# jesusdpa1/ssqueeze_rs

Measured on AMD Instinct MI355X. Metric: TF-bins/sec (ssq_stft, n_fft=1024), higher is better.
Workload: dtype f32

## Files before the change

ssqueeze_rs_amd/csrc/stft_fused.hip:

```cpp
#include "stft_fused_kernel.h"

namespace ssq {

struct Hi1024 {
  static constexpr int N = 1024, L = 64, NF = 513, W = 16, F = 16, PITCH = F + 1, THREADS = W * 64;
  static constexpr int PLANE = NF * PITCH;
  static constexpr int TILE_BYTES = (((2 * PLANE + F) * 4 + 15) / 16) * 16;
  static constexpr int EXH_ELEMS = 64 * 9;
  static constexpr int EXH_BYTES = W * EXH_ELEMS * 8;
  static constexpr int TAB_BYTES = N * 8;
  static constexpr int LDS_BYTES = TILE_BYTES + EXH_BYTES + 2 * TAB_BYTES;
  static constexpr int FRAC = 30, EMIN = -90;
  static_assert(LDS_BYTES <= 160 * 1024, "LDS budget");
};

__device__ __forceinline__ void rows_transpose4(float& r0, float& r1, float& r2, float& r3) {
  auto a = __builtin_amdgcn_permlane32_swap(__float_as_uint(r0), __float_as_uint(r2), false, false);
  auto b = __builtin_amdgcn_permlane32_swap(__float_as_uint(r1), __float_as_uint(r3), false, false);
  auto c = __builtin_amdgcn_permlane16_swap(a[0], b[0], false, false);
  auto d = __builtin_amdgcn_permlane16_swap(a[1], b[1], false, false);
  r0 = __uint_as_float(c[0]);
  r1 = __uint_as_float(c[1]);
  r2 = __uint_as_float(d[0]);
  r3 = __uint_as_float(d[1]);
}

template <bool EDGE, bool LEB, bool WKDBG = false>
__global__ __launch_bounds__(1024, 1) void stft_tx1024_kernel(StftDev<float> p) {
  using H = Hi1024;
  constexpr int THREADS = H::THREADS;
  using T = float;
  constexpr int N = H::N, L = H::L, NF = H::NF, F = H::F, PITCH = H::PITCH;
  __shared__ __attribute__((aligned(16))) unsigned char smem[H::LDS_BYTES];
  int* tile_re = reinterpret_cast<int*>(smem);
  float* col_scale = reinterpret_cast<float*>(tile_re + 2 * H::PLANE);
  cpx<T>* exch_all = reinterpret_cast<cpx<T>*>(smem + H::TILE_BYTES);
  cpx<T>* win_lds = reinterpret_cast<cpx<T>*>(smem + H::TILE_BYTES + H::EXH_BYTES);
  cpx<T>* tw1 = win_lds + N;
  cpx<T>* tw2 = tw1 + 256;

  const int tid = threadIdx.x;
  const int t = tid & 63;
  const int fl = __builtin_amdgcn_readfirstlane(tid >> 6);
  cpx<T>* exch = exch_all + fl * H::EXH_ELEMS;

  for (int i = tid; i < N; i += THREADS) win_lds[i] = p.win2[i];
  if (tid < 256) tw1[tid] = p.tw[((tid & 15) * (tid >> 4) * 4) & (N - 1)];
  for (int i = tid; i < 768; i += THREADS) tw2[i] = p.tw[((i & 255) * ((i >> 8) + 1)) & (N - 1)];
  constexpr long long CELL0 = WKDBG ? 0LL : 0x80000000LL;
  for (int i = tid; i < H::PLANE; i += THREADS) reinterpret_cast<long long*>(tile_re)[i] = CELL0;
  __syncthreads();
  const unsigned bid = blockIdx.x;
  if ((long long)bid >= p.total_tiles) return;

  const long long n_sig = p.total_tiles / p.tiles_per_signal;
  long long sig = (long long)(bid / (unsigned)p.tiles_per_signal);
  int jt = (int)(bid % (unsigned)p.tiles_per_signal);
  auto tile_frame0 = [&](int j) { return ((j < p.ta_n) ? p.ta0 + j : p.tb0 + (j - p.ta_n)) * F; };
  auto load_frame = [&](long long sg, int frame0, T (&xv)[16]) {
    const int frame = frame0 + fl;
    const T* xs = sig_base(p, sg);
    const long long pos0 = (long long)frame * p.hop - p.pad_left + t;
    if constexpr (!EDGE) {
#pragma unroll
      for (int q = 0; q < 16; ++q) xv[q] = xs[pos0 + L * q];
    } else {
      const bool valid = frame < p.n_frames;
      const long long first = pos0 - t;
      if (__all(valid && first >= 0 && first + N <= p.n_signal)) {
#pragma unroll
        for (int q = 0; q < 16; ++q) xv[q] = xs[pos0 + L * q];
      } else {
#pragma unroll
        for (int q = 0; q < 16; ++q) xv[q] = load_padded_flat(xs, pos0 + L * q, p.n_signal, p.padtype, valid);
      }
    }
  };
  T xn[16];
  load_frame(sig, tile_frame0(jt), xn);
  const cpx<T> twr_unused[3][16] = {};

  auto read_out = [&](long long rsig, int rframe0) {
    if constexpr (!EDGE && !WKDBG) {
      if ((p.n_frames & 1) == 0) {
        constexpr int RS2 = THREADS / (F / 2);
        const int fp = tid % (F / 2);
        const int k0 = tid / (F / 2);
        float4* __restrict__ og4 = reinterpret_cast<float4*>(p.out + rsig * (long long)NF * p.n_frames + rframe0 + 2 * fp +
                                                             (long long)k0 * p.n_frames);
        const long long gstep4 = (long long)RS2 * p.n_frames / 2;
        const T sc0 = col_scale[2 * fp], sc1 = col_scale[2 * fp + 1];
        long long* tc = reinterpret_cast<long long*>(tile_re) + k0 * PITCH + 2 * fp;
        auto sweep2 = [&](int j) {
          const long long c0 = tc[j * RS2 * PITCH], c1 = tc[j * RS2 * PITCH + 1];
          tc[j * RS2 * PITCH] = CELL0;
          tc[j * RS2 * PITCH + 1] = CELL0;
          const int r0 = (int)c0 ^ (int)0x80000000, r1 = (int)c1 ^ (int)0x80000000;
          const int i0 = (int)(c0 >> 32), i1 = (int)(c1 >> 32);
          const float4 val = make_float4((T)r0 * sc0, (T)i0 * sc0, (T)r1 * sc1, (T)i1 * sc1);
          typedef float vf4 __attribute__((ext_vector_type(4)));
          const vf4 nv = {val.x, val.y, val.z, val.w};
          __builtin_nontemporal_store(nv, reinterpret_cast<vf4*>(&og4[j * gstep4]));
        };
        constexpr int NFULL2 = NF / RS2;
#pragma unroll
        for (int j = 0; j < NFULL2; ++j) sweep2(j);
        if (k0 + NFULL2 * RS2 < NF) sweep2(NFULL2);
        return;
      }
    }
    constexpr int RSTEP = THREADS / F;
    const int f = tid % F;
    const int k0 = tid / F;
    cpx<T>* __restrict__ og = p.out + rsig * (long long)NF * p.n_frames + rframe0 + f + (long long)k0 * p.n_frames;
    const long long gstep = (long long)RSTEP * p.n_frames;
    const bool fvalid = EDGE ? (rframe0 + f < p.n_frames) : true;
    const T sc = col_scale[f];
    constexpr int NFULL = NF / RSTEP;
    long long* tc = reinterpret_cast<long long*>(tile_re) + k0 * PITCH + f;
    auto sweep = [&](int j) {
      const long long c = tc[j * RSTEP * PITCH];
      tc[j * RSTEP * PITCH] = CELL0;
      if constexpr (WKDBG) {
        if (fvalid) og[j * gstep] = cpx<T>{__int_as_float((int)c), __int_as_float((int)(c >> 32))};
        return;
      }
      const int ire = (int)c ^ (int)0x80000000;
      const int iim = (int)(c >> 32);
      if (fvalid) og[j * gstep] = cpx<T>{(T)ire * sc, (T)iim * sc};
    };
#pragma unroll
    for (int j = 0; j < NFULL; ++j) sweep(j);
    if (k0 + NFULL * RSTEP < NF) sweep(NFULL);
  };

  const int grid_n = (int)gridDim.x;
#pragma unroll 1
  while (true) {
    const int frame0 = tile_frame0(jt);
    const bool valid = EDGE ? (frame0 + fl < p.n_frames) : true;
    long long nsig = sig;
    int njt = jt + grid_n;
    while (njt >= p.tiles_per_signal) {
      njt -= p.tiles_per_signal;
      ++nsig;
    }
    const bool has_next = nsig < n_sig;
    cpx<T> v[16];
#pragma unroll
    for (int q = 0; q < 16; ++q) {
      const cpx<T> wq = win_lds[t + L * q];
      v[q] = {xn[q] * wq.x, xn[q] * wq.y};
    }

    fft_compute<T, 10, 0, false, false>(v, twr_unused, tw1, t);
    {
      cpx<T> nv[16];
      const int rbase = 9 * (t >> 4) + (t & 7);
#pragma unroll
      for (int ph = 0; ph < 2; ++ph) {
#pragma unroll
        for (int u = 0; u < 8; ++u) exch[9 * t + u] = v[8 * ph + u];
        frame_sync<false>();
        if (((t >> 3) & 1) == ph) {
#pragma unroll
          for (int q = 0; q < 16; ++q) nv[q] = exch[rbase + 36 * q];
        }
        frame_sync<false>();
      }
#pragma unroll
      for (int q = 0; q < 16; ++q) v[q] = nv[q];
    }
    if (has_next) load_frame(nsig, tile_frame0(njt), xn);
    fft_compute<T, 10, 1, false, false, true>(v, twr_unused, tw1, t);
    {
#pragma unroll
      for (int uh = 0; uh < 4; ++uh) {
        rows_transpose4(v[4 * uh + 0].x, v[4 * uh + 1].x, v[4 * uh + 2].x, v[4 * uh + 3].x);
        rows_transpose4(v[4 * uh + 0].y, v[4 * uh + 1].y, v[4 * uh + 2].y, v[4 * uh + 3].y);
      }
#define SSQ_SWAP(i, j)       \
  {                          \
    const cpx<T> t_ = v[i];  \
    v[i] = v[j];             \
    v[j] = t_;               \
  }
      SSQ_SWAP(1, 4) SSQ_SWAP(2, 8) SSQ_SWAP(3, 12) SSQ_SWAP(6, 9) SSQ_SWAP(7, 13) SSQ_SWAP(11, 14)
#undef SSQ_SWAP
    }
    fft_compute<T, 10, 2, false, false, true>(v, twr_unused, tw2 - 256, t);

    cpx<T> zp[9];
    {
      const int src = (L - t) & (L - 1);
      zp[8] = v[8];
      if (t == 0) {
#pragma unroll
        for (int j = 8; j < 15; ++j) v[j] = v[j + 1];
        v[15] = v[0];
      }
#pragma unroll
      for (int q = 0; q < 8; ++q) {
        zp[q].x = __shfl(v[15 - q].x, src);
        zp[q].y = __shfl(v[15 - q].y, src);
      }
      v[8] = zp[8];
    }

    {
      cpx<T> cv[9];
      int dstb[9];
      T wdbg[9];
      int kdbg[9];
      T l1 = 0.0f;
      constexpr int CELL = 8;
      const float lane_on = valid ? 1.0f : 0.0f;
      const float sfs0 = (float)t * p.sfs_step, sfs_q = (float)L * p.sfs_step;
      const int neg_last = -(p.n_freqs - 1);
#pragma unroll
      for (int q = 0; q < 9; ++q) {
        const cpx<T> zk = v[q], zn = zp[q];
        const cpx<T> S = {zk.x + zn.x, zk.y - zn.y};
        const cpx<T> dS = {zk.y + zn.y, zn.x - zk.x};
        const float den = S.x * S.x + S.y * S.y;
        const float num = dS.y * S.x - dS.x * S.y;
        const float pd = num * __builtin_amdgcn_rcpf(den * p.two_pi_eff);
        const float d = (sfs0 + (float)q * sfs_q) - pd;
        const float w = fabsf(d);
        float m = fma_clamp01(den, p.keep_big, p.keep_bias) * fma_clamp01(d, 0.0f, 1.0f);
        if (EDGE) m *= lane_on;
        if (q == 8) m *= (t == 0) ? 1.0f : 0.0f;
        const cpx<T> c = LEB ? cpx<T>{p.leb_unit * m, 0.0f} : cpx<T>{S.x * m, S.y * m};
        cv[q] = c;
        int kneg = cvt_floor_i32(__builtin_fmaf(-w, p.inv_dw, 0.5f));
        kneg = kneg < neg_last ? neg_last : kneg;
        dstb[q] = __mul24(kneg, -(PITCH * CELL)) + fl * CELL;
        l1 += fabsf(c.x) + fabsf(c.y);
        if constexpr (WKDBG) {
          wdbg[q] = w;
          kdbg[q] = (m != 0.0f) ? -kneg : -1;
        }
      }
      const T tot = frame_allreduce<T, L, false>(l1, t, nullptr, t) * p.dw;
      T scale, inv_scale;
      column_scale<T, H::FRAC, H::EMIN>(tot, p.dw, scale, inv_scale);
      if (t == 0 && valid) col_scale[fl] = inv_scale;
      char* ptile = reinterpret_cast<char*>(tile_re);
      if constexpr (WKDBG) {
#pragma unroll
        for (int q = 0; q < 9; ++q) {
          if ((q < 8 || t == 0) && valid) {
            const unsigned lo = (unsigned)__float_as_int(wdbg[q]), hi = (unsigned)__float_as_int((float)kdbg[q]);
            reinterpret_cast<unsigned long long*>(ptile)[(t + L * q) * PITCH + fl] = ((unsigned long long)hi << 32) | lo;
          }
        }
      } else {
#pragma unroll
        for (int q = 0; q < 9; ++q) {
          const int ia = cvt_round_i32(cv[q].x * scale);
          const int ib = LEB ? 0 : cvt_round_i32(cv[q].y * scale);
          if (q < 8 || t == 0) {
            if (LEB) {
              atomicAdd(reinterpret_cast<unsigned*>(ptile + dstb[q]), (unsigned)ia);
            } else {
              const unsigned hi = (unsigned)(ib + (ia >> 31));
              atomicAdd(reinterpret_cast<unsigned long long*>(ptile + dstb[q]),
                        ((unsigned long long)hi << 32) | (unsigned)ia);
            }
          }
        }
      }
    }
    __syncthreads();
    read_out(sig, frame0);
    __syncthreads();
    if (!has_next) break;
    sig = nsig;
    jt = njt;
  }
}

template <typename T>
bool fused_supported(int n_fft) {
  return n_fft >= 64 && n_fft <= 4096 && (n_fft & (n_fft - 1)) == 0;
}

template <typename T, int LOGN>
static hipError_t launch_one(const StftDev<T>& p0, int cu_count, long long batch, hipStream_t stream) {
  using C = FusedCfg<T, LOGN>;
  int per_cu = (160 * 1024) / C::LDS_BYTES;
  if (per_cu < 1) per_cu = 1;
  if (per_cu * C::W > 32) per_cu = 32 / C::W;
  bool tx1024 = false;
  if constexpr (sizeof(T) == 4 && LOGN == 10) tx1024 = (p0.out_kind == 0 || p0.out_kind == 3) && p0.n_eff == C::N;
  const int TF = tx1024 ? Hi1024::F : C::F;
  const long long span = (long long)TF * p0.hop;
  const int tps_all = (p0.n_frames + TF - 1) / TF;
  long long lo = (p0.pad_left + span - 1) / span;
  long long hi_num = p0.n_signal - C::N - (long long)(TF - 1) * p0.hop + p0.pad_left;
  long long hi = hi_num >= 0 ? hi_num / span + 1 : 0;
  const long long full = p0.n_frames / TF;
  if (hi > full) hi = full;
  if (lo > tps_all) lo = tps_all;
  if (hi < lo) hi = lo;
  const long long blocks_one_wave = (long long)cu_count * (tx1024 ? 1 : per_cu);
  bool single_launch = (long long)tps_all * batch <= 4 * blocks_one_wave;
  if (const char* e = std::getenv("SSQ_SINGLE_LAUNCH")) single_launch = std::atoi(e) != 0;
  for (int edge = single_launch ? 1 : 0; edge < 2; ++edge) {
    StftDev<T> p = p0;
    if (single_launch) {
      p.ta0 = 0;
      p.ta_n = tps_all;
      p.tb0 = 0;
      p.tiles_per_signal = tps_all;
    } else if (!edge) {
      p.ta0 = (int)lo;
      p.ta_n = (int)(hi - lo);
      p.tb0 = 0;
      p.tiles_per_signal = p.ta_n;
    } else {
      p.ta0 = 0;
      p.ta_n = (int)lo;
      p.tb0 = (int)hi;
      p.tiles_per_signal = (int)lo + (tps_all - (int)hi);
    }
    p.total_tiles = (long long)p.tiles_per_signal * batch;
    if (p.total_tiles <= 0) continue;
    long long blocks = (long long)cu_count * per_cu;
    if (blocks > p.total_tiles) blocks = p.total_tiles;
    const dim3 g((unsigned)blocks), b(C::W * 64);
    if constexpr (sizeof(T) == 4 && LOGN == 10) {
      if (tx1024) {
        long long nb = cu_count;
        if (nb > p.total_tiles) nb = p.total_tiles;
        const dim3 gh((unsigned)nb), bh(Hi1024::THREADS);
        if (p.out_kind == 3) {
          if (edge) hipLaunchKernelGGL((stft_tx1024_kernel<true, false, true>), gh, bh, 0, stream, p);
          else hipLaunchKernelGGL((stft_tx1024_kernel<false, false, true>), gh, bh, 0, stream, p);
        } else if (p.squeezing == 1) {
          if (edge) hipLaunchKernelGGL((stft_tx1024_kernel<true, true>), gh, bh, 0, stream, p);
          else hipLaunchKernelGGL((stft_tx1024_kernel<false, true>), gh, bh, 0, stream, p);
        } else {
          if (edge) hipLaunchKernelGGL((stft_tx1024_kernel<true, false>), gh, bh, 0, stream, p);
          else hipLaunchKernelGGL((stft_tx1024_kernel<false, false>), gh, bh, 0, stream, p);
        }
        const hipError_t eh = hipGetLastError();
        if (eh != hipSuccess) return eh;
        continue;
      }
    }
    if (p.out_kind == 0 && p.squeezing == 1) {
      if (edge) hipLaunchKernelGGL((stft_fused_kernel<T, LOGN, true, true, true>), g, b, 0, stream, p);
      else hipLaunchKernelGGL((stft_fused_kernel<T, LOGN, true, false, true>), g, b, 0, stream, p);
    } else if (p.out_kind == 0) {
      if (edge) hipLaunchKernelGGL((stft_fused_kernel<T, LOGN, true, true, false>), g, b, 0, stream, p);
      else hipLaunchKernelGGL((stft_fused_kernel<T, LOGN, true, false, false>), g, b, 0, stream, p);
    } else if (p.out_kind == 3) {
      if (edge) hipLaunchKernelGGL((stft_fused_kernel<T, LOGN, true, true, false, true>), g, b, 0, stream, p);
      else hipLaunchKernelGGL((stft_fused_kernel<T, LOGN, true, false, false, true>), g, b, 0, stream, p);
    } else {
      if (edge) hipLaunchKernelGGL((stft_fused_kernel<T, LOGN, false, true, false>), g, b, 0, stream, p);
      else hipLaunchKernelGGL((stft_fused_kernel<T, LOGN, false, false, false>), g, b, 0, stream, p);
    }
    const hipError_t e = hipGetLastError();
    if (e != hipSuccess) return e;
  }
  return hipSuccess;
}

template <typename T>
int fused_tile_frames(int n_fft) {
  switch (n_fft) {
    case 64: return FusedCfg<T, 6>::F;
    case 128: return FusedCfg<T, 7>::F;
    case 256: return FusedCfg<T, 8>::F;
    case 512: return FusedCfg<T, 9>::F;
    case 1024: return FusedCfg<T, 10>::F;
    case 2048: return FusedCfg<T, 11>::F;
    case 4096: return FusedCfg<T, 12>::F;
  }
  return 0;
}

template <typename T>
hipError_t launch_stft_fused(const StftDev<T>& p, int n_fft, int cu_count, long long batch, hipStream_t stream) {
  if (p.n_eff != n_fft) return launch_stft_anylen<T>(p, n_fft, cu_count, batch, stream);
  switch (n_fft) {
    case 64: return launch_one<T, 6>(p, cu_count, batch, stream);
    case 128: return launch_one<T, 7>(p, cu_count, batch, stream);
    case 256: return launch_one<T, 8>(p, cu_count, batch, stream);
    case 512: return launch_one<T, 9>(p, cu_count, batch, stream);
    case 1024: return launch_one<T, 10>(p, cu_count, batch, stream);
    case 2048: return launch_one<T, 11>(p, cu_count, batch, stream);
    case 4096: return launch_one<T, 12>(p, cu_count, batch, stream);
  }
  return hipErrorInvalidValue;
}

template bool fused_supported<float>(int);
template bool fused_supported<double>(int);
template int fused_tile_frames<float>(int);
template int fused_tile_frames<double>(int);
template hipError_t launch_stft_fused<float>(const StftDev<float>&, int, int, long long, hipStream_t);
template hipError_t launch_stft_fused<double>(const StftDev<double>&, int, int, long long, hipStream_t);

}
```

Measured before the change: 291.6 billion.

## Merge interior and edge tile passes of tx1024 STFT kernel into one launch

Moves the tx1024 tile loop into a device function and has the interior-tile kernel run the edge-tile pass afterwards in the same launch, reusing the LDS window/twiddle setup. This drops the second kernel launch, its repeated LDS initialisation and the tail gap between the two launches. The cost is instantiating the EDGE path inside the interior kernel, which may raise register pressure or code size. The lane id is recomputed via mbcnt for the second pass.

```diff
diff --git a/ssqueeze_rs_amd/csrc/stft_fused.hip b/ssqueeze_rs_amd/csrc/stft_fused.hip
--- a/ssqueeze_rs_amd/csrc/stft_fused.hip
+++ b/ssqueeze_rs_amd/csrc/stft_fused.hip
@@ -25,13 +25,18 @@
   r3 = __uint_as_float(d[1]);
 }
 
-template <bool EDGE, bool LEB, bool WKDBG = false>
-__global__ __launch_bounds__(1024, 1) void stft_tx1024_kernel(StftDev<float> p) {
+struct Tx1024Range {
+  int ta0, ta_n, tb0, tps;
+  long long total;
+};
+
+template <bool EDGE, bool LEB, bool WKDBG, bool SECOND = false>
+__device__ __forceinline__ void tx1024_tiles(const StftDev<float>& p, const Tx1024Range& r, unsigned char* smem,
+                                             const unsigned bid, const int grid_n, const int wave = 0) {
   using H = Hi1024;
   constexpr int THREADS = H::THREADS;
   using T = float;
   constexpr int N = H::N, L = H::L, NF = H::NF, F = H::F, PITCH = H::PITCH;
-  __shared__ __attribute__((aligned(16))) unsigned char smem[H::LDS_BYTES];
   int* tile_re = reinterpret_cast<int*>(smem);
   float* col_scale = reinterpret_cast<float*>(tile_re + 2 * H::PLANE);
   cpx<T>* exch_all = reinterpret_cast<cpx<T>*>(smem + H::TILE_BYTES);
@@ -39,24 +44,21 @@
   cpx<T>* tw1 = win_lds + N;
   cpx<T>* tw2 = tw1 + 256;
 
-  const int tid = threadIdx.x;
+  int tid = threadIdx.x;
+  if constexpr (SECOND) {
+    int lane = __builtin_amdgcn_mbcnt_hi(~0u, __builtin_amdgcn_mbcnt_lo(~0u, 0u));
+    asm volatile("" : "+v"(lane));
+    tid = (wave << 6) | lane;
+  }
   const int t = tid & 63;
-  const int fl = __builtin_amdgcn_readfirstlane(tid >> 6);
+  const int fl = SECOND ? wave : __builtin_amdgcn_readfirstlane(tid >> 6);
   cpx<T>* exch = exch_all + fl * H::EXH_ELEMS;
-
-  for (int i = tid; i < N; i += THREADS) win_lds[i] = p.win2[i];
-  if (tid < 256) tw1[tid] = p.tw[((tid & 15) * (tid >> 4) * 4) & (N - 1)];
-  for (int i = tid; i < 768; i += THREADS) tw2[i] = p.tw[((i & 255) * ((i >> 8) + 1)) & (N - 1)];
   constexpr long long CELL0 = WKDBG ? 0LL : 0x80000000LL;
-  for (int i = tid; i < H::PLANE; i += THREADS) reinterpret_cast<long long*>(tile_re)[i] = CELL0;
-  __syncthreads();
-  const unsigned bid = blockIdx.x;
-  if ((long long)bid >= p.total_tiles) return;
-
-  const long long n_sig = p.total_tiles / p.tiles_per_signal;
-  long long sig = (long long)(bid / (unsigned)p.tiles_per_signal);
-  int jt = (int)(bid % (unsigned)p.tiles_per_signal);
-  auto tile_frame0 = [&](int j) { return ((j < p.ta_n) ? p.ta0 + j : p.tb0 + (j - p.ta_n)) * F; };
+
+  const long long n_sig = r.total / r.tps;
+  long long sig = (long long)(bid / (unsigned)r.tps);
+  int jt = (int)(bid % (unsigned)r.tps);
+  auto tile_frame0 = [&](int j) { return ((j < r.ta_n) ? r.ta0 + j : r.tb0 + (j - r.ta_n)) * F; };
   auto load_frame = [&](long long sg, int frame0, T (&xv)[16]) {
     const int frame = frame0 + fl;
     const T* xs = sig_base(p, sg);
@@ -134,15 +136,14 @@
     if (k0 + NFULL * RSTEP < NF) sweep(NFULL);
   };
 
-  const int grid_n = (int)gridDim.x;
 #pragma unroll 1
   while (true) {
     const int frame0 = tile_frame0(jt);
     const bool valid = EDGE ? (frame0 + fl < p.n_frames) : true;
     long long nsig = sig;
     int njt = jt + grid_n;
-    while (njt >= p.tiles_per_signal) {
-      njt -= p.tiles_per_signal;
+    while (njt >= r.tps) {
+      njt -= r.tps;
       ++nsig;
     }
     const bool has_next = nsig < n_sig;
@@ -280,6 +281,37 @@
   }
 }
 
+template <bool EDGE, bool LEB, bool WKDBG = false>
+__global__ __launch_bounds__(1024, 1) void stft_tx1024_kernel(StftDev<float> p, int edge_tps) {
+  using H = Hi1024;
+  constexpr int THREADS = H::THREADS, N = H::N;
+  using T = float;
+  __shared__ __attribute__((aligned(16))) unsigned char smem[H::LDS_BYTES];
+  cpx<T>* win_lds = reinterpret_cast<cpx<T>*>(smem + H::TILE_BYTES + H::EXH_BYTES);
+  cpx<T>* tw1 = win_lds + N;
+  cpx<T>* tw2 = tw1 + 256;
+  const int tid = threadIdx.x;
+  for (int i = tid; i < N; i += THREADS) win_lds[i] = p.win2[i];
+  if (tid < 256) tw1[tid] = p.tw[((tid & 15) * (tid >> 4) * 4) & (N - 1)];
+  for (int i = tid; i < 768; i += THREADS) tw2[i] = p.tw[((i & 255) * ((i >> 8) + 1)) & (N - 1)];
+  constexpr long long CELL0 = WKDBG ? 0LL : 0x80000000LL;
+  for (int i = tid; i < H::PLANE; i += THREADS) reinterpret_cast<long long*>(smem)[i] = CELL0;
+  __syncthreads();
+  const unsigned bid = blockIdx.x;
+  const int wave = __builtin_amdgcn_readfirstlane(tid >> 6);
+  const int grid_n = (int)gridDim.x;
+  const Tx1024Range r = {p.ta0, p.ta_n, p.tb0, p.tiles_per_signal, p.total_tiles};
+  if ((long long)bid < r.total) tx1024_tiles<EDGE, LEB, WKDBG>(p, r, smem, bid, grid_n);
+  if constexpr (!EDGE) {
+    if (edge_tps > 0) {
+      const long long n_sig = p.total_tiles / p.tiles_per_signal;
+      const Tx1024Range re = {0, p.ta0, p.ta0 + p.ta_n, edge_tps, (long long)edge_tps * n_sig};
+      const int grid_e = re.total < (long long)grid_n ? (int)re.total : grid_n;
+      if ((long long)bid < re.total) tx1024_tiles<true, LEB, WKDBG, true>(p, re, smem, bid, grid_e, wave);
+    }
+  }
+}
+
 template <typename T>
 bool fused_supported(int n_fft) {
   return n_fft >= 64 && n_fft <= 4096 && (n_fft & (n_fft - 1)) == 0;
@@ -306,6 +338,7 @@
   const long long blocks_one_wave = (long long)cu_count * (tx1024 ? 1 : per_cu);
   bool single_launch = (long long)tps_all * batch <= 4 * blocks_one_wave;
   if (const char* e = std::getenv("SSQ_SINGLE_LAUNCH")) single_launch = std::atoi(e) != 0;
+  const int tps_int = (int)(hi - lo), tps_edge = (int)lo + (tps_all - (int)hi);
   for (int edge = single_launch ? 1 : 0; edge < 2; ++edge) {
     StftDev<T> p = p0;
     if (single_launch) {
@@ -315,14 +348,14 @@
       p.tiles_per_signal = tps_all;
     } else if (!edge) {
       p.ta0 = (int)lo;
-      p.ta_n = (int)(hi - lo);
+      p.ta_n = tps_int;
       p.tb0 = 0;
       p.tiles_per_signal = p.ta_n;
     } else {
       p.ta0 = 0;
       p.ta_n = (int)lo;
       p.tb0 = (int)hi;
-      p.tiles_per_signal = (int)lo + (tps_all - (int)hi);
+      p.tiles_per_signal = tps_edge;
     }
     p.total_tiles = (long long)p.tiles_per_signal * batch;
     if (p.total_tiles <= 0) continue;
@@ -331,18 +364,21 @@
     const dim3 g((unsigned)blocks), b(C::W * 64);
     if constexpr (sizeof(T) == 4 && LOGN == 10) {
       if (tx1024) {
+        const bool merged = !single_launch && tps_int > 0;
+        if (merged && edge) continue;
+        const int etps = merged ? tps_edge : 0;
         long long nb = cu_count;
         if (nb > p.total_tiles) nb = p.total_tiles;
         const dim3 gh((unsigned)nb), bh(Hi1024::THREADS);
         if (p.out_kind == 3) {
-          if (edge) hipLaunchKernelGGL((stft_tx1024_kernel<true, false, true>), gh, bh, 0, stream, p);
-          else hipLaunchKernelGGL((stft_tx1024_kernel<false, false, true>), gh, bh, 0, stream, p);
+          if (edge) hipLaunchKernelGGL((stft_tx1024_kernel<true, false, true>), gh, bh, 0, stream, p, 0);
+          else hipLaunchKernelGGL((stft_tx1024_kernel<false, false, true>), gh, bh, 0, stream, p, etps);
         } else if (p.squeezing == 1) {
-          if (edge) hipLaunchKernelGGL((stft_tx1024_kernel<true, true>), gh, bh, 0, stream, p);
-          else hipLaunchKernelGGL((stft_tx1024_kernel<false, true>), gh, bh, 0, stream, p);
+          if (edge) hipLaunchKernelGGL((stft_tx1024_kernel<true, true>), gh, bh, 0, stream, p, 0);
+          else hipLaunchKernelGGL((stft_tx1024_kernel<false, true>), gh, bh, 0, stream, p, etps);
         } else {
-          if (edge) hipLaunchKernelGGL((stft_tx1024_kernel<true, false>), gh, bh, 0, stream, p);
-          else hipLaunchKernelGGL((stft_tx1024_kernel<false, false>), gh, bh, 0, stream, p);
+          if (edge) hipLaunchKernelGGL((stft_tx1024_kernel<true, false>), gh, bh, 0, stream, p, 0);
+          else hipLaunchKernelGGL((stft_tx1024_kernel<false, false>), gh, bh, 0, stream, p, etps);
         }
         const hipError_t eh = hipGetLastError();
         if (eh != hipSuccess) return eh;
```

Result: no change. 289.0 billion (-0.9%).
